# rland93/rrtplanner

Measured on AMD Instinct MI355X. Metric: RRT* nodes-expanded/s on 1024x1024 Perlin grid; achieved HBM GB/s, higher is better.
Workload: dtype int16x2 coordinates / u32 squared distances / f64 costs; 1 GPU; BASELINE.json configs[1]: RRT* 1024x1024 n=50000 r_rewire=64; queries_per_gpu=1, total_queries=1, n=50000, unfinished_queries=0, cus_per_query=129, pipelined=True, team_fallbacks=0, collective_library=librccl.so.1

## Files before the change

### rrtplanner_amd/csrc/kernels_tu.hip

```cpp
#include <hip/hip_runtime.h>

#ifndef RRT_TU
#error "kernels_tu.hip is compiled once per unit: pass -DRRT_TU=k (the Makefile's TUS)"
#endif

#if RRT_TU == 1
#include "rrt_pipe.h"

#elif RRT_TU == 4
#define RRT_PIPE_LARGE_TU
#include "rrt_pipe.h"

#elif RRT_TU == 2
#include "rrt_dubins_block.h"
#include "rrt_serial.h"
namespace rrtdev {
template __global__ void rrt_expand_kernel<false, true>(BatchView);
}

#elif RRT_TU == 3
#include "rrt_serial.h"
namespace rrtdev {
template __global__ void rrt_expand_kernel<false, false>(BatchView);
template __global__ void rrt_expand_kernel<true, false>(BatchView);
// ... 7 lines not shown
#include "rrt_routes.h"

#elif RRT_TU == 7
#include "rrt_keep.h"

#elif RRT_TU == 8
#include "rrt_seed.h"
#include "rrt_pose_seed.h"

#elif RRT_TU == 9
#include "rrt_pose_goals.h"
#include "rrt_pose_keep.h"
#include "rrt_pose_routes.h"

#elif RRT_TU == 0
#include "rrt_reroot.h"
#include "rrt_relax.h"
#include "rrt_pose_relax.h"
#include "rrt_pose_reroot.h"

#elif RRT_TU == -1
#include "rrt_pose_field.h"

#else
#include "rrt_block.h"
namespace rrtdev {
#define K(G, BSM, PIPE, INF) template __global__ void rrt_expand_block_kernel<G, BSM, PIPE, INF>(BatchView);
#define S(G, BSM, INF)                                                        \
    template __global__ void rrt_block_commit_kernel<G, BSM, INF>(BatchView); \
    template __global__ void rrt_block_work_kernel<G, BSM, INF>(BatchView);
#define RRT_PASTE_(a, b) a##b
#define RRT_PASTE(a, b) RRT_PASTE_(a, b)
RRT_PASTE(RRT_UNIT_, RRT_TU)(K, S)
#undef K
#undef S
}
#endif
```

### rrtplanner_amd/csrc/rrt_block.h

```cpp
#pragma once

#include "rrt_go2goal.h"
#include "rrt_cell_stream.h"

namespace rrtdev {

constexpr int BS = 16;

#ifndef RRT_PIPE_LAG
#define RRT_PIPE_LAG 2
#endif
#ifndef RRT_PIPE_LAG_SMALL
#define RRT_PIPE_LAG_SMALL 1
#endif
#ifndef RRT_PIPE_LAG_INF
#define RRT_PIPE_LAG_INF 2
#endif
constexpr unsigned long long TEAM_TIMEOUT_TICKS = 50000000ull;

typedef unsigned long long u64;
typedef __attribute__((address_space(1))) uint32_t gu32;
typedef __attribute__((address_space(1))) u64 gu64;
#define RRT_RLX_AGENT __ATOMIC_RELAXED, __HIP_MEMORY_SCOPE_AGENT

// ... 103 lines not shown
    int32_t i, j, nsoln, vbest_soln, pad0, pad1;
    double cmin_soln, c_ell;
};

template <int BSM>
__device__ __forceinline__ void block_scan_step(u32x4 quad, const uint32_t (&xs16)[BSM], uint32_t (&best)[BSM], uint32_t tag0) {
    const uint32_t n0 = quad.x << 4, n1 = quad.y << 4, n2 = quad.z << 4, n3 = quad.w << 4;
#pragma unroll
    for (int k = 0; k < BSM; ++k) {
        const uint32_t k0 = key16(n0, xs16[k], tag0), k1 = key16(n1, xs16[k], tag0 + 1), k2 = key16(n2, xs16[k], tag0 + 2),
                       k3 = key16(n3, xs16[k], tag0 + 3);
        best[k] = min(min(best[k], k0), min(min(k1, k2), k3));
    }
}

struct GSlot {
    double c1, c2;
    uint32_t i1, i2;
    uint32_t hits, nlist;
    uint32_t nn_d2, nn_idx;
    uint32_t pad[2];
    uint32_t x1, x2;
    uint32_t nn_xy, nn_vlo, nn_vhi;
};
struct GCtl {
    double lbc;
    uint32_t lbi, consume;
    double bound;
};

union BlkWords {
    BlkState b;
    u64 w[5];
};

struct ParRound {
    u64 acc_opt, aprev[NPMAX];
    uint32_t list[NWAVE];
    uint32_t accs[64];
    uint32_t count;
    int32_t jp0[NPMAX];
};

template <bool PIPE, bool INF, int BSM>
struct PipeShape {
    static constexpr int LAG = PIPE ? (INF ? RRT_PIPE_LAG_INF : (BSM >= 16 ? RRT_PIPE_LAG_SMALL : RRT_PIPE_LAG)) : 0;
    static_assert(LAG <= NPMAX, "a record carries masks for NPMAX blocks in flight");
    static constexpr int NP = LAG > 0 ? LAG : 1;
    static constexpr int NSLOT = PIPE ? LAG + 1 : 1;
};

template <int G, int BSM, bool PIPE, bool INF>
struct BlockLds {
    static constexpr int SB = BSM * G, NP = PipeShape<PIPE, INF, BSM>::NP;
    alignas(16) u32x2 nnx[(BSM <= BS ? BSM : 1) * NWAVE];
    alignas(16) BRec brec[PIPE ? 2 : 1][SB];
    uint32_t xq_next[PIPE ? 2 : 1][PIPE ? 64 : 1];
    uint32_t pre_state[2];
    alignas(16) BSlot bslots[2 * NWAVE];
    alignas(16) BlkState blk;
    alignas(16) unsigned long long statred[SB * 5];
    uint32_t xq_lds[SB];
    double newcost[SB];
    alignas(16) ParRound par;
    uint32_t xqp_lds[PIPE ? NP : 1][PIPE ? 64 : 1];
    double prevcost[PIPE ? NP : 1][PIPE ? 64 : 1];
    uint32_t help_n[NWAVE], help_x[NWAVE];
    uint32_t help_any;
    uint32_t tick;
    uint32_t slots[BSM >= 16 ? NWAVE : 1][64];
    alignas(16) GSlot gslot[NWAVE];
    alignas(16) GCtl gctl[BSM];
    alignas(8) uint16_t plist[(PIPE && BSM < 16) ? BSM : 1][PL_MAX];
    uint32_t oq_cnt[(PIPE && BSM < 16) ? BSM : 1], oq_ovf;
    uint32_t qhist[16], qstage2;
#ifdef RRT_STAMPS
    unsigned long long dbg[16];
#endif
};

constexpr int ROLE_ALL = 0, ROLE_COMMIT = 1, ROLE_WORK = 2;


template <int G, int BSM, bool PIPE, bool INF, int ROLE, int CW = NWAVE>
__device__ __forceinline__ void rrt_block_body(BatchView bv, BlockLds<G, BSM, PIPE, INF> &L) {
    static_assert(CW == NWAVE || ROLE == ROLE_COMMIT, "only a committer runs with fewer waves");
    constexpr int NTG = CW * 64;
    static_assert(G >= 1 && G <= TEAM_MAX && BSM >= 1 && BSM * G <= 64, "team size");
    constexpr bool WIDE = BSM > BS;
    static_assert(!PIPE || G > 1, "a pipeline needs a team");
    static_assert(PIPE == (ROLE != ROLE_ALL), "roles are the halves of a pipelined team");
    constexpr int LAG = PipeShape<PIPE, INF, BSM>::LAG, NP = PipeShape<PIPE, INF, BSM>::NP, NSLOT = PipeShape<PIPE, INF, BSM>::NSLOT;
    constexpr int SB = BSM * G;
#ifndef RRT_CG16
#define RRT_CG16 2
#endif
    constexpr int CG = (BSM >= 16) ? (ROLE == ROLE_COMMIT ? 2 : RRT_CG16) : 1;
#ifndef RRT_BLOCK_SCATTER
#define RRT_BLOCK_SCATTER 1
#endif
    constexpr bool SCATTER = RRT_BLOCK_SCATTER && BSM >= 16;
    extern __shared__ __attribute__((aligned(16))) unsigned char smem[];
    auto &nnx = L.nnx;
    auto &brec = L.brec;
    auto &xq_next = L.xq_next;
    auto &pre_state = L.pre_state;
    auto &bslots = L.bslots;
    auto &blk = L.blk;
    auto &statred = L.statred;
    auto &xq_lds = L.xq_lds;
    auto &newcost = L.newcost;
    auto &par = L.par;
    auto &xqp_lds = L.xqp_lds;
    auto &prevcost = L.prevcost;
    auto &gslot = L.gslot;
    auto &gctl = L.gctl;
    constexpr int WPS = BSM >= 16 ? 1 : NWAVE / BSM;
    constexpr bool FASTL = PIPE && WPS > 1;
    const int t = (int)threadIdx.x, lane = t & 63, wave = t >> 6;
    int q = (int)blockIdx.x, g_ = 0;
    if (G > 1) {
        q = (int)blockIdx.x % bv.team_qpad;
        g_ = (int)blockIdx.x / bv.team_qpad + bv.member0;
        if (q >= bv.Q) return;
// ... 44 lines not shown
    const int lds_chunks = bv.lds_chunks;
    const int lds_nodes = lds_chunks * CHUNK;
    const uint32_t r2 = D->r2_rewire, goal_d2 = D->goal_d2;
    const uint32_t xs = pack_xy(D->xs[0], D->xs[1]), xg = pack_xy(D->xg[0], D->xg[1]);
    const int ub_offset = D->ub_offset, ub_count = D->ub_count;
    const int cshift = D->cell_shift, ncy = D->ncy, ccap = D->cell_cap, ncells = D->ncx * D->ncy;
    u32x4 *cellrec = reinterpret_cast<u32x4 *>(bv.cellrec) + (size_t)q * (size_t)bv.rec_stride;
    uint32_t *cellcnt_g = bv.cellcnt + (size_t)q * (size_t)MAX_CELLS;
    const bool cells_on = star || BSM >= 16;
    const uint32_t r2h = star ? r2 : (cells_on ? (uint32_t)((2 << cshift) * (2 << cshift)) : 0u);
    int rad = 0;
    if (r2h > 0) {
        rad = (r2h >= (1u << 23)) ? 4096 : (int)sqrtf((float)(r2h - 1));
        while (rad > 0 && (uint32_t)(rad * rad) > r2h - 1) --rad;
        while ((uint32_t)((rad + 1) * (rad + 1)) <= r2h - 1) ++rad;
    }

    RRT_LDS uint32_t *nodes_lds = (RRT_LDS uint32_t *)smem;
    const RRT_LDS u32x4 *nodes_lds4 = (const RRT_LDS u32x4 *)smem;
    RRT_LDS uint32_t *cellcnt = (RRT_LDS uint32_t *)(smem + (size_t)lds_chunks * CHUNK * sizeof(uint32_t));

    int i = D->i, j = D->j;
    int nsoln = D->nsoln, vbest_soln = D->vbest_soln;
    double cmin_soln = D->cmin_soln;
    int i_switch = D->i_switch;
    int status = ST_RUNNING;
#ifdef RRT_STAMPS
    unsigned long long cyc[6] = {D->cyc[0], D->cyc[1], D->cyc[2], D->cyc[3], D->cyc[4], D->cyc[5]};
    unsigned long long tstamp = __builtin_amdgcn_s_memtime();
    unsigned long long wcyc_acc = 0, wcyc_los = 0;
    auto &dbg = L.dbg;
    if (t < 16) dbg[t] = 0;
    unsigned long long dbgt = __builtin_amdgcn_s_memtime();
#ifdef RRT_STAMPS_LIGHT
#define DBGT(k)                                                      \
    do {                                                             \
        if (((RRT_STAMPS_LIGHT) >> (k)) & 1) {                       \
            unsigned long long now_ = __builtin_amdgcn_s_memtime();  \
            if (t == 0) dbg[k] += now_ - dbgt;                       \
            dbgt = now_;                                             \
        }                                                            \
    } while (0)
#else
#define DBGT(k)                                                  \
    do {                                                         \
        unsigned long long now_ = __builtin_amdgcn_s_memtime();  \
        if (t == 0) dbg[k] += now_ - dbgt;                       \
        dbgt = now_;                                             \
    } while (0)
#endif
#else
#define DBGT(k) \
    do {        \
    } while (0)
#endif

#if defined(RRT_STAMPS)
#define TSMARK(ep, ev)                                                                                          \
    do {                                                                                                        \
        if ((int)(ep) >= RRT_TS_BASE && (int)(ep) < RRT_TS_BASE + 32 && lane == 0) D->ts[((int)(ep) - RRT_TS_BASE) * 16 + (ev)] = wall_clock64(); \
    } while (0)
#else
#define TSMARK(ep, ev) \
    do {               \
    } while (0)
#endif
// ... 137 lines not shown
                    if (base + 3 >= jlim) cur.w = node0;
                }
                block_scan_step<BSA>(cur, xs16, best, (uint32_t)c << 2);
                cur = nxt;
            }
        }
    };

    constexpr int32_t ST_FLAG_RESTART = 1, ST_FLAG_STOP = 2;
    const bool pipe_inf = PIPE && informed;
    int nprev = 0;
    int void_turns = 0;
    bool prefetched = false;
    bool prefetched_smp = false;
    int bsel = 0;
    auto publish_state = [&](uint32_t ep, int32_t flags) {
        if (lane == 0) {
            BlkWords u;
            u.b.i = i;
            u.b.j = j;
            u.b.nsoln = nsoln;
            u.b.vbest_soln = vbest_soln;
            u.b.pad0 = 0;
            u.b.pad1 = flags;
            u.b.cmin_soln = cmin_soln;
            u.b.c_ell = c_ell;
#pragma unroll
            for (int w = 0; w < 5; ++w) __hip_atomic_store(t_state + (size_t)(ep % NSLOT) * 8 + w, u.w[w], RRT_RLX_AGENT);
        }
        asm volatile("s_waitcnt vmcnt(0)" ::: "memory");
        if (lane == 0) __hip_atomic_store(t_go, ep, RRT_RLX_AGENT);
        if (!grid_nn) __builtin_amdgcn_fence(__ATOMIC_ACQUIRE, "agent");
    };
    if (PIPE && SH == 2) {
        if (shift1) {
            if (wave == 0) xqp_lds[0][lane] = (i + lane < n) ? at32(samples, (uint32_t)(i + lane)) : 0u;
            i += SB;
            epoch = 1;
            nprev = 1;
        }
        __syncthreads();
    }
    while ((pipe_inf && g > 0) || i < n) {
        const int i0 = i, j0 = j;
        int nb = (n - i0) < SB ? (n - i0) : SB;
        const bool ell = informed && nsoln > 0;
        bool void_blk = false;
        if (nb <= 0) {
            nb = 0;
            void_blk = true;
        }
        if (ell) {
            if (i_switch == n) i_switch = i0;
            const int u0i = i0 - ub_offset;
            if (ub == nullptr || u0i < 0 || u0i + nb > ub_count) {
                if (pipe_inf && g > 0) {
                    nb = 0;
                    void_blk = true;
                } else {
                    status = ST_NEED_UB;
                    if (pipe_inf && wave == 0) publish_state(epoch + 1, ST_FLAG_STOP);
                    break;
                }
            }
        }
        ++epoch;
// ... 220 lines not shown
        for (int k = 0; k < 16; ++k) D->wcyc[16 * g + k] = dbg[k];
#endif
}

template <int G, int BSM, bool PIPE, bool INF>
__global__ __launch_bounds__(TPB) void rrt_expand_block_kernel(BatchView bv) {
    __shared__ BlockLds<G, BSM, PIPE, INF> L;
    if constexpr (PIPE) {
#if defined(RRT_ONLY_ROLE) && RRT_ONLY_ROLE == 1
        rrt_block_body<G, BSM, PIPE, INF, ROLE_COMMIT>(bv, L);
#elif defined(RRT_ONLY_ROLE) && RRT_ONLY_ROLE == 2
        rrt_block_body<G, BSM, PIPE, INF, ROLE_WORK>(bv, L);
#else
        if ((int)blockIdx.x < bv.team_qpad) rrt_block_body<G, BSM, PIPE, INF, ROLE_COMMIT>(bv, L);
        else rrt_block_body<G, BSM, PIPE, INF, ROLE_WORK>(bv, L);
#endif
    } else {
        rrt_block_body<G, BSM, PIPE, INF, ROLE_ALL>(bv, L);
    }
}

template <int G, int BSM, bool INF>
__global__ __launch_bounds__(512) void rrt_block_commit_kernel(BatchView bv) {
    __shared__ BlockLds<G, BSM, true, INF> L;
    rrt_block_body<G, BSM, true, INF, ROLE_COMMIT, 8>(bv, L);
}

template <int G, int BSM, bool INF>
__global__ __launch_bounds__(TPB) void rrt_block_work_kernel(BatchView bv) {
    __shared__ BlockLds<G, BSM, true, INF> L;
    rrt_block_body<G, BSM, true, INF, ROLE_WORK>(bv, L);
}

}

#include "rrt_block_variants.def"
```

### rrtplanner_amd/csrc/rrt_block_handover.inc

```

        if (PIPE && g > 0) {
#ifdef RRT_STAMPS
            if (t == 0 && g <= 64) {
                const unsigned long long dres = __builtin_amdgcn_s_memtime() - wres0;
                if (dres > 26000ull) D->dbg2[192 + g - 1] += 1;
                if (dres > 32000ull) D->dbg2[256 + g - 1] += 1;
                if (dres > 40000ull) D->dbg2[320 + g - 1] += 1;
                if (dres > D->dbg2[384 + g - 1]) D->dbg2[384 + g - 1] = dres;
            }
#endif
            DBGT(0);
            const int i_next = i0 + nb + (SH - 1) * SB;
            const bool more = i_next < n;
            const uint32_t ep_take = epoch + (uint32_t)(SH - 1) - (uint32_t)LAG;
            const bool take = (int)epoch + SH - 1 > LAG && (more || pipe_inf);
            if (wave == 0) {
                if (!void_blk) {
                    const RRT_LDS u64 *src = (const RRT_LDS u64 *)&brec[0][wg * BSM];
                    gu64 *dst = t_rec + (size_t)(epoch % NSLOT) * 64 * BREC_WORDS + (size_t)wg * BSM * BREC_WORDS;
                    for (int w = lane; w < BSM * BREC_WORDS; w += 64) __hip_atomic_store(dst + w, src[w], RRT_RLX_AGENT);
                    asm volatile("s_waitcnt vmcnt(0)" ::: "memory");
                }
                if (lane == 0) __hip_atomic_store(my_arrive(), epoch, RRT_RLX_AGENT);
                if (g == 1) TSMARK(epoch, 5);
                if (g == 8) TSMARK(epoch, 8);
            }
            pre_i = -1;
            if (!informed && more && !grid_nn) {
                pre_i = i_next;
                pre_j = j0;
                const int nbn = (n - pre_i) < SB ? (n - pre_i) : SB;
                pre_xv = lane < nbn ? at32(samples, (uint32_t)(pre_i + lane)) : 0u;
                uint32_t xsn[BSA];
#pragma unroll
                for (int k = 0; k < BSA; ++k) {
                    const int sk = wg * BSM + k;
                    uint32_t X = (uint32_t)__builtin_amdgcn_readlane((int)pre_xv, sk);
                    if (sk >= nbn) X = (uint32_t)__builtin_amdgcn_readlane((int)pre_xv, 0);
                    xsn[k] = X << 4;
                    pre_best[k] = NONE;
                }
                scan_steps(0, pre_j / CHUNK, pre_j, xsn, pre_best);
            }
            if (wave == 0) {
                bool ok = true;
                if (SH == 2) {
                    xqp_lds[NP - 1][lane] = xv;
                    xqp_lds[0][lane] = more ? at32(samples, (uint32_t)(i0 + nb + lane)) : 0u;
                } else {
#pragma unroll
                    for (int p2 = NP - 1; p2 > 0; --p2) xqp_lds[p2][lane] = xqp_lds[p2 - 1][lane];
                    xqp_lds[0][lane] = xv;
                }
                DBGT(1);
                if (take) {
                    ok = team_wait(t_go, ep_take, t_fail);
                    if (g == 1) TSMARK(epoch, 6);
                    if (g == 8) TSMARK(epoch, 9);
// ... 24 lines not shown
                    if (cells_on) __hip_atomic_fetch_add(&cellcnt[cell_of(Xn)], 1u, __ATOMIC_RELAXED, __HIP_MEMORY_SCOPE_WORKGROUP);
                }
                j = jn;
                if (pipe_inf) {
                    nsoln = unis32(u.b.nsoln);
                    vbest_soln = unis32(u.b.vbest_soln);
                    cmin_soln = unif64(u.b.cmin_soln);
                    c_ell = unif64(u.b.c_ell);
                    if ((u.b.pad1 & ST_FLAG_RESTART) != 0) {
                        __syncthreads();
                        if (wave == 0) {
                            const bool ok2 = team_wait(t_go, epoch, t_fail);
                            if (lane == 0) blk.pad0 = ok2 ? 0 : 1;
                        }
                        __syncthreads();
                        if (blk.pad0 != 0) {
                            team_failed = true;
                            break;
                        }
                        BlkWords u2;
#pragma unroll
                        for (int w = 0; w < 5; ++w) u2.w[w] = __hip_atomic_load(t_state + (size_t)(epoch % NSLOT) * 8 + w, RRT_RLX_AGENT);
                        if ((u2.b.pad1 & ST_FLAG_STOP) != 0) break;
                        i = unis32(u.b.i);
                        nprev = 0;
                    }
                }
            }
            __syncthreads();
            if (wave == 0 && g == 1) TSMARK(epoch, 7);
            if (wave == 0 && g == 8) TSMARK(epoch, 10);
            DBGT(3);
            epoch += (uint32_t)(SH - 1);
            continue;
        }

        if (G > 1 && !PIPE && g > 0) {
            if (wave == 0) {
                const RRT_LDS u64 *src = (const RRT_LDS u64 *)&brec[0][g * BSM];
                for (int w = lane; w < BSM * BREC_WORDS; w += 64) __hip_atomic_store(t_rec + (size_t)g * BSM * BREC_WORDS + w, src[w], RRT_RLX_AGENT);
                asm volatile("s_waitcnt vmcnt(0)" ::: "memory");
                if (lane == 0) __hip_atomic_store(t_arrive + 32 * g, epoch, RRT_RLX_AGENT);
            }
            pre_i = -1;
            if (!informed && i0 + nb < n && !grid_nn) {
                pre_i = i0 + nb;
                pre_j = j0;
                const int nbn = (n - pre_i) < SB ? (n - pre_i) : SB;
                pre_xv = lane < nbn ? samples[pre_i + lane] : 0u;
                uint32_t xsn[BSA];
#pragma unroll
                for (int k = 0; k < BSA; ++k) {
                    const int sk = g * BSM + k;
                    uint32_t X = (uint32_t)__builtin_amdgcn_readlane((int)pre_xv, sk);
                    if (sk >= nbn) X = (uint32_t)__builtin_amdgcn_readlane((int)pre_xv, 0);
                    xsn[k] = X << 4;
                    pre_best[k] = NONE;
                }
                scan_steps(0, pre_j / CHUNK, pre_j, xsn, pre_best);
            }
            if (wave == 0) {
                const bool ok = team_wait(t_go, epoch, t_fail);
                if (!grid_nn) {
                    __builtin_amdgcn_fence(__ATOMIC_ACQUIRE, "agent");
                    asm volatile("s_waitcnt vmcnt(0)" ::: "memory");
                }
// ... 26 lines not shown
```

### rrtplanner_amd/csrc/rrt_block_worker.inc

```

        if (worker && !void_blk) {
        uint32_t xs16[BSA];
#pragma unroll
        for (int k = 0; k < BSA; ++k) {
            const int sk = wg * BSM + k;
            uint32_t X = (uint32_t)__builtin_amdgcn_readlane((int)xv, sk);
            if (sk >= nb) X = (uint32_t)__builtin_amdgcn_readlane((int)xv, 0);
            xs16[k] = X << 4;
        }

        const int nsteps = (j0 + CHUNK - 1) / CHUNK;
        if (!grid_nn) {
            uint32_t best[BSA];
            int c_first = 0;
            if (G > 1 && pre_i == i0) {
                c_first = pre_j / CHUNK;
#pragma unroll
                for (int k = 0; k < BSA; ++k) best[k] = pre_best[k];
            } else {
#pragma unroll
                for (int k = 0; k < BSA; ++k) best[k] = NONE;
            }
            scan_steps(c_first, nsteps, j0, xs16, best);
            uint32_t gd = NONE, gi = NONE;
// ... 378 lines not shown
                            pnn[p2] = __ballot(dp < d2s);
                            pr[p2] = __ballot(star && dp < r2);
                            pdup[p2] = __ballot(xop == Xk);
                        }
                    }
                }
#ifdef RRT_STAMPS
                gs2 = __builtin_amdgcn_s_memtime();
#endif
                if (star) {
                    if (overflow) {
                        nnear = 0;
                        amin = 0.0f;
                        snapshot_parent(Xk, j0, false, cnear_s, pc, pi, nnear, ntests, tcells);
                    } else if (tt.i1 != NONE) {
                        if (!tested3) los_wave2(og, H, tx1, tt.i2 != NONE ? tx2 : Xk, tt.i2 != NONE, Xk, lane, ok1, cc1, ok2, cc2);
                        ntests += 1;
                        tcells += (uint32_t)cc1;
                        if (ok1) {
                            pc = tt.c1;
                            pi = tt.i1;
                        } else if (tt.i2 != NONE) {
                            ntests += 1;
                            tcells += (uint32_t)cc2;
                            if (ok2) {
                                pc = tt.c2;
                                pi = tt.i2;
                            } else {
                                consume = true;
                                lbc = tt.c2;
                                lbi = tt.i2 + 1;
                            }
                        }
                    }
                }
            }
#ifdef RRT_STAMPS
            if (lead) gs3 = __builtin_amdgcn_s_memtime();
#endif
            if (star) {
                if (lead && lane == 0) {
                    GCtl c;
                    c.lbc = lbc;
                    c.lbi = lbi;
                    c.consume = (act && consume) ? 1u : 0u;
                    c.bound = cnear_s;
                    gctl[sl] = c;
                }
                __syncthreads();
                const GCtl c = gctl[sl];
                auto qbin = [](double cn, double lo, double hi) -> int {
                    const double w = hi - lo;
                    if (!(w > 0.0)) return 0;
                    const int b = (int)((cn - lo) * (16.0 / w));
                    return b < 0 ? 0 : (b > 15 ? 15 : b);
                };
                bool by_queue = false;
                if constexpr (GQ) {
                    if (rad < 64) {
                        RRT_LDS u32x4 *const oq = (RRT_LDS u32x4 *)&brec[1][0] + (size_t)sl * OQCAP;
#ifdef RRT_STAMPS
                        unsigned long long qt0 = __builtin_amdgcn_s_memtime(), qt1 = qt0, qt2 = qt0, qt3 = qt0, qt4 = qt0;
#endif
                        if (c.consume != 0u) {
                            const float boundf = screen_of(c.bound);
                            float am = FINF;
// ... 383 lines not shown
```

### rrtplanner_amd/csrc/rrt_engine.hip

```cpp
#include "rrt_engine.h"
#include "rrt_prims.h"

static thread_local std::string g_last_error;

constexpr int RRT_GRID_FAST = 2048;
constexpr int RRT_GRID_LARGE = 4096;
constexpr int RRT_GRID_MAX = 32767;

struct BlockVariant {
    int G, BSM;
    bool pipe, inf;
    block_kernel_fn one, commit, work;
};
static const BlockVariant g_block_variants[] = {
#define K(G, BSM, PIPE, INF) {G, BSM, PIPE, INF, rrt_expand_block_kernel<G, BSM, PIPE, INF>, nullptr, nullptr},
#define S(G, BSM, INF) {G, BSM, true, INF, nullptr, rrt_block_commit_kernel<G, BSM, INF>, rrt_block_work_kernel<G, BSM, INF>},
#define U(k) RRT_UNIT_##k(K, S)
    RRT_BLOCK_UNITS(U)
#undef U
#undef S
#undef K
};

static const BlockVariant *find_variant(int team, bool pipe, bool inf, bool wide, bool split) {
    for (const BlockVariant &r : g_block_variants)
        if (r.G == team && r.pipe == pipe && r.inf == inf && (r.BSM > 16) == wide && (r.commit != nullptr) == split) return &r;
    return nullptr;
}

static size_t block_kernel_static_lds(int team) {
    hipFuncAttributes a{};
    size_t worst = 0;
    for (const BlockVariant &r : g_block_variants)
        for (block_kernel_fn k : {r.one, r.commit, r.work}) {
            if (!k || r.G > team) continue;
            if (hipFuncGetAttributes(&a, reinterpret_cast<const void *>(k)) != hipSuccess) return 16384;
            worst = a.sharedSizeBytes > worst ? a.sharedSizeBytes : worst;
        }
    return (worst + 255) & ~(size_t)255;
}

void drop_keep_views(rrt_batch *b, int32_t q) {
    for (size_t k = 0; k < b->keep_alive.size(); ++k)
        if ((q < 0 || (size_t)q == k) && b->keep_alive[k] >= 0) {
            b->keep_alive[k] = -1;
            b->ran_gen[k] = 0;
            b->ran_og[k] = nullptr;
        }
}

static hipError_t raise_dynamic_lds(int device, const void *kern, int bytes) {
    static std::mutex mu;
    static std::vector<std::tuple<int, const void *, int>> have;
    std::lock_guard<std::mutex> lock(mu);
    for (auto &t : have)
        if (std::get<0>(t) == device && std::get<1>(t) == kern) {
            if (std::get<2>(t) >= bytes) return hipSuccess;
            const hipError_t e = hipFuncSetAttribute(kern, hipFuncAttributeMaxDynamicSharedMemorySize, bytes);
            if (e == hipSuccess) std::get<2>(t) = bytes;
            return e;
        }
    const hipError_t e = hipFuncSetAttribute(kern, hipFuncAttributeMaxDynamicSharedMemorySize, bytes);
    if (e == hipSuccess) have.emplace_back(device, kern, bytes);
    return e;
}

int fail(rrt_ctx *ctx, int code, const char *fmt, ...) {
// ... 771 lines not shown

extern "C" int rrt_batch_launch(rrt_batch *b) {
    if (!b) return fail(nullptr, RRT_E_ARG, "rrt_batch_launch: NULL");
    rrt_ctx *ctx = b->ctx;
    for (int q = 0; q < b->Q; ++q)
        if (b->grow_n[(size_t)q] >= 0 && b->h_desc[(size_t)q].status == ST_RUNNING &&
            (b->grow_gen[(size_t)q] != ctx->grid_gen || b->grow_og[(size_t)q] != ctx->og))
            return fail(ctx, RRT_E_ARG, "rrt_batch_launch: the context's grid was replaced since query %d was seeded by rrt_batch_grow (grid generation %llu then, "
                        "%llu now): its seed belongs to the other grid (rrt_batch_rearm drops the grow)", q, (unsigned long long)b->grow_gen[(size_t)q],
                        (unsigned long long)ctx->grid_gen);
    b->drop_routes();
    drop_keep_views(b);
    if (!ctx->og) return fail(ctx, RRT_E_NOGRID, "rrt_batch_launch: no grid");
    if (b->gridW != ctx->W || b->gridH != ctx->H) return fail(ctx, RRT_E_ARG, "rrt_batch_launch: grid changed shape");
    HIPCHK(ctx, hipSetDevice(ctx->device));
    if (!b->one_cu_once) b->ms_before = 0.f;
    LaunchPlan &p = b->last;
    if (const int rc = plan_launch(b, p); rc != RRT_OK) return rc;
    for (int q = 0; q < b->Q; ++q)
        if (b->h_desc[(size_t)q].status == ST_RUNNING) {
            b->ran_gen[(size_t)q] = ctx->grid_gen;
            b->ran_og[(size_t)q] = ctx->og;
        }
    BatchView v = make_view(b);
    v.team_qpad = p.qpad;
    v.shifts = p.shifts;
    if (p.shifts == 2) v.spill_stride = b->spill_stride2;
    v.lds_chunks = p.lds_chunks;
    if (p.split) {
        if (!ctx->stream2) HIPCHK(ctx, hipStreamCreateWithFlags(&ctx->stream2, hipStreamNonBlocking));
        if (!b->ev_fork) HIPCHK(ctx, hipEventCreateWithFlags(&b->ev_fork, hipEventDisableTiming));
        if (!b->ev_join) HIPCHK(ctx, hipEventCreateWithFlags(&b->ev_join, hipEventDisableTiming));
    }
    for (block_kernel_fn k : {p.kern, p.split ? p.row->commit : nullptr, p.split ? p.row->work : nullptr})
        if (k && p.lds_bytes) HIPCHK(ctx, raise_dynamic_lds(ctx->device, reinterpret_cast<const void *>(k), (int)p.lds_bytes));
    const dim3 ig((unsigned)((b->bitmap_words + 255) / 256 > 64 ? 64 : (b->bitmap_words + 255) / 256), (unsigned)b->Q);
    hipLaunchKernelGGL(rrt_init_kernel<0>, ig, dim3(256), 0, ctx->stream, v);
    if (p.team > 1) HIPCHK(ctx, hipMemsetAsync(b->d_team, 0, (size_t)b->Q * TEAM_BYTES, ctx->stream));
    HIPCHK(ctx, hipEventRecord(b->ev0, ctx->stream));
    if (p.split) {
        HIPCHK(ctx, hipEventRecord(b->ev_fork, ctx->stream));
        HIPCHK(ctx, hipStreamWaitEvent(ctx->stream2, b->ev_fork, 0));
        hipLaunchKernelGGL(p.row->commit, dim3((unsigned)p.qpad), dim3(512), p.lds_bytes, ctx->stream2, v);
        BatchView vw = v;
        vw.member0 = 1;
        hipLaunchKernelGGL(p.row->work, dim3((unsigned)(p.qpad * p.team * p.shifts)), dim3(TPB), p.lds_bytes, ctx->stream, vw);
        HIPCHK(ctx, hipEventRecord(b->ev_join, ctx->stream2));
        HIPCHK(ctx, hipStreamWaitEvent(ctx->stream, b->ev_join, 0));
    } else {
        hipLaunchKernelGGL(p.kern, dim3(p.grid), dim3(TPB), p.lds_bytes, ctx->stream, v);
    }
    HIPCHK(ctx, hipEventRecord(b->ev1, ctx->stream));
    HIPCHK(ctx, hipGetLastError());
    b->timed = true;
    return RRT_OK;
}

extern "C" int rrt_batch_sync(rrt_batch *b) {
    if (!b) return fail(nullptr, RRT_E_ARG, "rrt_batch_sync: NULL");
    rrt_ctx *ctx = b->ctx;
    HIPCHK(ctx, hipSetDevice(ctx->device));
    HIPCHK(ctx, hipMemcpyAsync(b->h_desc.data(), b->d_desc, (size_t)b->Q * sizeof(QDesc), hipMemcpyDeviceToHost, ctx->stream));
    HIPCHK(ctx, wait_stream_spin(ctx->stream));
    cu_release(ctx->device, b->claimed_cus);
    b->claimed_cus = 0;
#ifdef RRT_STAMPS
    if (getenv("RRT_STAMPS_DUMP")) {
        const QDesc &d0 = b->h_desc[0];
        fprintf(stderr, "dbg2 groups of slow blocks (> 32 k) [count, own stream, first barrier, nearest + LoS, top-2 LoS, tail, consume, empty ball]:");
        for (int m = 0; m < 8; ++m) fprintf(stderr, " %llu", d0.dbg2[m]);
        fprintf(stderr, "\ndbg2 groups of the other blocks:");
        for (int m = 8; m < 16; ++m) fprintf(stderr, " %llu", d0.dbg2[m]);
        fprintf(stderr, "\ndbg2 groups queue, fast [count, gctl barrier, pricing, barrier, tests, barrier, queue entries, time before]:");
        for (int m = 16; m < 24; ++m) fprintf(stderr, " %llu", d0.dbg2[m]);
        fprintf(stderr, "\ndbg2 groups queue, slow (> 30 k at the last barrier):");
        for (int m = 24; m < 32; ++m) fprintf(stderr, " %llu", d0.dbg2[m]);
        fprintf(stderr, "\ndbg2 missing-polls:");
        for (int m = 0; m < 64; ++m) fprintf(stderr, " %llu", d0.dbg2[m]);
        fprintf(stderr, "\ndbg2 last-to-arrive:");
// ... 713 lines not shown
```

### rrtplanner_amd/csrc/rrt_kernel_abi.h

```cpp
#pragma once

#include <hip/hip_runtime.h>
#include <stddef.h>
#include <stdint.h>

namespace rrtdev {

constexpr int TPB = 1024;
constexpr int NWAVE = TPB / 64;
constexpr int CHUNK = TPB * 4;
constexpr int MAX_LDS_CHUNKS = 8;
constexpr int WSLOTS = 3;
constexpr int WCAP = 64 * WSLOTS;
constexpr uint32_t NONE = 0xffffffffu;

typedef uint32_t u32x4 __attribute__((ext_vector_type(4)));

#ifndef RRT_TS_BASE
#define RRT_TS_BASE 300
#endif

enum : int32_t { ST_DONE = 0, ST_NEED_UB = 1, ST_UNREACHABLE = -2, ST_TEAM_FAIL = -3, ST_RUNNING = 100, ST_IDLE = 101 };

struct QDesc {
// ... 376 lines not shown
    uint8_t *item_h;
    int32_t x0, y0, w, h;
    int32_t heading_lo, heading_hi;
    int32_t run;
    int32_t *vertex;
    double *cost;
    int32_t *heading_out;
};
enum : int { POSE_FIELD_CELLS = 0, POSE_FIELD_BUCKETS_SEEN = 1, POSE_FIELD_WORDS = 2, POSE_FIELD_SWEEPS = 3, POSE_FIELD_STATS = 4 };

struct PoseRerootView {
    const uint32_t *nodes;
    const int32_t *parent;
    const uint8_t *heading;
    const int32_t *id;
    int32_t j, root;
    uint32_t *f_nodes;
    int32_t *f_parent;
    uint8_t *f_heading;
    int32_t *f_id;
};

template <bool RW, bool DUB = false>
__global__ __launch_bounds__(TPB) void rrt_expand_kernel(BatchView bv);
__global__ __launch_bounds__(TPB) void rrt_pipe_kernel(BatchView bv);
__global__ __launch_bounds__(TPB) void rrt_pipe_large_kernel(BatchView bv);
__global__ __launch_bounds__(TPB) void rrt_dubins_block_kernel(BatchView bv);
template <int G, int BSM, bool PIPE, bool INF>
__global__ __launch_bounds__(TPB) void rrt_expand_block_kernel(BatchView bv);
template <int G, int BSM, bool INF>
__global__ __launch_bounds__(512) void rrt_block_commit_kernel(BatchView bv);
template <int G, int BSM, bool INF>
__global__ __launch_bounds__(TPB) void rrt_block_work_kernel(BatchView bv);
__global__ __launch_bounds__(TPB) void rrt_goals_kernel(GoalsView gv);
__global__ __launch_bounds__(TPB) void rrt_goals_large_kernel(GoalsView gv);
__global__ __launch_bounds__(TPB) void rrt_pose_goals_kernel(PoseGoalsView pv);
__global__ __launch_bounds__(FIELD_TPB) void rrt_field_kernel(FieldView fv);
__global__ __launch_bounds__(FIELD_TPB) void rrt_field_large_kernel(FieldView fv);
__global__ __launch_bounds__(ROUTE_TPB) void rrt_route_depth_kernel(RoutesView rv);
__global__ __launch_bounds__(TPB) void rrt_route_scan_kernel(const int32_t *in, int64_t *out, int32_t m);
__global__ __launch_bounds__(ROUTE_TPB) void rrt_route_fill_kernel(RoutesView rv, int32_t with_len);
__global__ __launch_bounds__(TPB) void rrt_route_cut_kernel(RoutesView rv);
__global__ __launch_bounds__(TPB) void rrt_route_cut_large_kernel(RoutesView rv);
__global__ __launch_bounds__(ROUTE_TPB) void rrt_route_pack_kernel(RoutesView rv);
__global__ __launch_bounds__(KEEP_TPB) void rrt_keep_edge_kernel(KeepView kv);
__global__ __launch_bounds__(KEEP_TPB) void rrt_keep_edge_large_kernel(KeepView kv);
__global__ __launch_bounds__(KEEP_TPB) void rrt_keep_jump_kernel(const uint8_t *ok, const int32_t *anc, uint8_t *ok2, int32_t *anc2, int32_t j);
__global__ __launch_bounds__(TPB) void rrt_keep_compact_kernel(KeepCompact kc);
__global__ __launch_bounds__(KEEP_TPB) void rrt_keep_remap_kernel(int32_t *vertex, const int32_t *live_id, int32_t m, int32_t count);
__global__ __launch_bounds__(POSE_KEEP_TPB) void rrt_pose_keep_edge_kernel(PoseKeepView kv);
__global__ __launch_bounds__(POSE_KEEP_TPB) void rrt_pose_keep_gather_kernel(const uint8_t *heading, const int32_t *live_id, const int32_t *count,
                                                                            uint8_t *live_heading, int32_t j);
__global__ __launch_bounds__(POSE_ROUTE_TPB) void rrt_pose_route_fill_kernel(PoseRoutesView pr);
__global__ __launch_bounds__(POSE_ROUTE_TPB) void rrt_pose_route_leg_kernel(PoseRoutesView pr);
__global__ __launch_bounds__(POSE_ROUTE_TPB) void rrt_pose_route_length_kernel(PoseRoutesView pr);
__global__ __launch_bounds__(POSE_ROUTE_TPB) void rrt_pose_route_points_kernel(PoseRoutesView pr);
__global__ __launch_bounds__(POSE_CUT_TPB) void rrt_pose_route_cut_kernel(PoseCutView pc);
__global__ __launch_bounds__(POSE_CUT_TPB) void rrt_pose_route_pack_kernel(PoseCutView pc);
__global__ __launch_bounds__(SEED_TPB) void rrt_seed_rank_kernel(SeedView sv);
__global__ __launch_bounds__(SEED_TPB) void rrt_seed_parent_kernel(SeedView sv);
__global__ __launch_bounds__(SEED_TPB) void rrt_seed_install_kernel(SeedView sv);
__global__ __launch_bounds__(SEED_TPB) void rrt_seed_bitmap_kernel(SeedView sv);
__global__ __launch_bounds__(SEED_TPB) void rrt_seed_records_kernel(SeedRecords sr);
__global__ __launch_bounds__(SEED_TPB) void rrt_pose_seed_heading_kernel(uint8_t *heading, const uint8_t *live_heading, int32_t j0, int32_t node_stride);

__global__ __launch_bounds__(REROOT_TPB) void rrt_reroot_path_kernel(RerootView rv);
// ... 34 lines not shown
```

Baseline: 6.664 million nodes/s.

## Let split-team workers resolve ahead and patch results after the committer catches up

Adds a work-ahead variant of the pipelined worker kernel for the 64-member, BSM=1, non-informed split team. Workers take the next sample without waiting for the committer's state. When the committed state arrives, they patch their nearest/parent/rewire record using the newly inserted nodes, with a small LOS batch. If the patch cannot be done cheaply (too many new nodes, hard constraint, or overflow), they redo the block. The host picks this kernel when the rewire radius is between 16 and 64. The aim is to hide committer latency, at the cost of extra catch-up work and possible redo rounds.

```diff
diff --git a/rrtplanner_amd/csrc/kernels_tu.hip b/rrtplanner_amd/csrc/kernels_tu.hip
--- a/rrtplanner_amd/csrc/kernels_tu.hip
+++ b/rrtplanner_amd/csrc/kernels_tu.hip
@@ -63,6 +63,9 @@
 #define RRT_PASTE_(a, b) a##b
 #define RRT_PASTE(a, b) RRT_PASTE_(a, b)
 RRT_PASTE(RRT_UNIT_, RRT_TU)(K, S)
+#if RRT_TU == 22
+template __global__ void rrt_block_work_ahead_kernel<TEAM_MAX, 1, false>(BatchView);
+#endif
 #undef K
 #undef S
 }
diff --git a/rrtplanner_amd/csrc/rrt_block.h b/rrtplanner_amd/csrc/rrt_block.h
--- a/rrtplanner_amd/csrc/rrt_block.h
+++ b/rrtplanner_amd/csrc/rrt_block.h
@@ -159,6 +159,17 @@
 union BlkWords {
     BlkState b;
     u64 w[5];
+};
+
+constexpr uint32_t AH_T1 = 1u, AH_T2 = 2u;
+constexpr uint32_t AH_HARD = 4u;
+constexpr uint32_t AH_OVERFLOW = 8u;
+struct AheadSlot {
+    double c1, c2;
+    uint32_t i1, i2;
+    uint32_t cc1, cc2;
+    uint32_t st;
+    uint32_t redo;
 };
 
 struct ParRound {
@@ -209,7 +220,7 @@
 constexpr int ROLE_ALL = 0, ROLE_COMMIT = 1, ROLE_WORK = 2;
 
 
-template <int G, int BSM, bool PIPE, bool INF, int ROLE, int CW = NWAVE>
+template <int G, int BSM, bool PIPE, bool INF, int ROLE, int CW = NWAVE, bool AHEAD = false>
 __device__ __forceinline__ void rrt_block_body(BatchView bv, BlockLds<G, BSM, PIPE, INF> &L) {
     static_assert(CW == NWAVE || ROLE == ROLE_COMMIT, "only a committer runs with fewer waves");
     constexpr int NTG = CW * 64;
@@ -217,6 +228,7 @@
     constexpr bool WIDE = BSM > BS;
     static_assert(!PIPE || G > 1, "a pipeline needs a team");
     static_assert(PIPE == (ROLE != ROLE_ALL), "roles are the halves of a pipelined team");
+    static_assert(!AHEAD || (ROLE == ROLE_WORK && !INF && BSM == 1 && G == TEAM_MAX), "only the workers of the split team of 64 resolve ahead");
     constexpr int LAG = PipeShape<PIPE, INF, BSM>::LAG, NP = PipeShape<PIPE, INF, BSM>::NP, NSLOT = PipeShape<PIPE, INF, BSM>::NSLOT;
     constexpr int SB = BSM * G;
 #ifndef RRT_CG16
@@ -327,6 +339,7 @@
     auto &dbg = L.dbg;
     if (t < 16) dbg[t] = 0;
     unsigned long long dbgt = __builtin_amdgcn_s_memtime();
+    [[maybe_unused]] unsigned long long ah_go = 0;
 #ifdef RRT_STAMPS_LIGHT
 #define DBGT(k)                                                      \
     do {                                                             \
@@ -530,6 +543,10 @@
         if (lane == 0) __hip_atomic_store(t_go, ep, RRT_RLX_AGENT);
         if (!grid_nn) __builtin_amdgcn_fence(__ATOMIC_ACQUIRE, "agent");
     };
+    const bool ahead = AHEAD && SH == 2 && grid_nn && rad < 64;
+    bool early = false;
+    static_assert(!AHEAD || sizeof(AheadSlot) <= sizeof(L.newcost), "the catch-up's notes fit the committer's cost array");
+    [[maybe_unused]] RRT_LDS AheadSlot *const ah = AHEAD ? (RRT_LDS AheadSlot *)&newcost[0] : nullptr;
     if (PIPE && SH == 2) {
         if (shift1) {
             if (wave == 0) xqp_lds[0][lane] = (i + lane < n) ? at32(samples, (uint32_t)(i + lane)) : 0u;
@@ -816,6 +833,12 @@
     rrt_block_body<G, BSM, true, INF, ROLE_WORK>(bv, L);
 }
 
+template <int G, int BSM, bool INF>
+__global__ __launch_bounds__(TPB) void rrt_block_work_ahead_kernel(BatchView bv) {
+    __shared__ BlockLds<G, BSM, true, INF> L;
+    rrt_block_body<G, BSM, true, INF, ROLE_WORK, NWAVE, true>(bv, L);
+}
+
 }
 
 #include "rrt_block_variants.def"
diff --git a/rrtplanner_amd/csrc/rrt_block_handover.inc b/rrtplanner_amd/csrc/rrt_block_handover.inc
--- a/rrtplanner_amd/csrc/rrt_block_handover.inc
+++ b/rrtplanner_amd/csrc/rrt_block_handover.inc
@@ -10,10 +10,224 @@
             }
 #endif
             DBGT(0);
+            if constexpr (AHEAD) {
+                if (early) {
+                    early = false;
+                    if ((int)epoch - 1 > LAG) {
+                        const uint32_t ep_due = epoch - 1u - (uint32_t)LAG;
+                        DBGT(1);
+                        if (wave == 0) {
+                            const bool ok = team_wait(t_go, ep_due, t_fail);
+                            if (lane == 0) blk.pad0 = ok ? 0 : 1;
+                        }
+                        __syncthreads();
+                        DBGT(2);
+#ifdef RRT_STAMPS
+                        ah_go = __builtin_amdgcn_s_memtime();
+#endif
+                        if (blk.pad0 != 0) {
+                            team_failed = true;
+                            break;
+                        }
+                        BlkWords u;
+#pragma unroll
+                        for (int w = 0; w < 5; ++w) u.w[w] = __hip_atomic_load(t_state + (size_t)(ep_due % NSLOT) * 8 + w, RRT_RLX_AGENT);
+                        const int jn = unis32(u.b.j);
+                        if (t < jn - j0) {
+                            const uint32_t Xn = ld_u32<COH>(&at32(nodes_g, (uint32_t)(j0 + t)));
+                            if (j0 + t < lds_nodes) nodes_lds[j0 + t] = Xn;
+                            if (cells_on) __hip_atomic_fetch_add(&cellcnt[cell_of(Xn)], 1u, __ATOMIC_RELAXED, __HIP_MEMORY_SCOPE_WORKGROUP);
+                        }
+                        j = jn;
+                        if (wave == 0) {
+                            const int sidx = wg * BSM;
+                            const uint32_t Xk = (uint32_t)__builtin_amdgcn_readlane((int)xv, sidx);
+                            BRec &r = brec[0][sidx];
+                            const uint32_t st = uni32(ah->st);
+                            const int m = sidx < nb ? jn - j0 : 0;
+                            uint32_t redo = (m > 128 || (m > 0 && (st & AH_OVERFLOW) != 0u)) ? 1u : 0u;
+#ifdef RRT_STAMPS
+                            uint32_t lost = 0;
+#endif
+                            if (m > 0 && redo == 0u) {
+                                const uint32_t id0 = (uint32_t)(j0 + lane), id1 = id0 + 64u;
+                                const bool v0 = (int)id0 < jn, v1 = (int)id1 < jn;
+                                const uint32_t X0 = ld_u32<COH>(&at32(nodes_g, v0 ? id0 : 0u)), X1 = ld_u32<COH>(&at32(nodes_g, v1 ? id1 : 0u));
+                                const double V0 = ld_f64<COH>(&at32(vcost, v0 ? id0 : 0u)), V1 = ld_f64<COH>(&at32(vcost, v1 ? id1 : 0u));
+                                const uint32_t e0 = dist2(X0, Xk), e1 = dist2(X1, Xk);
+                                const bool dupn = __ballot((v0 && X0 == Xk) || (v1 && X1 == Xk)) != 0;
+                                uint32_t kd = v0 ? e0 : NONE, ki = v0 ? id0 : NONE;
+                                if (v1 && e1 < kd) {
+                                    kd = e1;
+                                    ki = id1;
+                                }
+                                wave_min_key_idx(kd, ki);
+                                uint32_t d2s = uni32(r.d2s), vs = uni32(r.vs), los_s = uni32(r.los_s), nnear = uni32(r.nnear);
+                                double Vs = unif64(r.Vs), pc = unif64(r.pc);
+                                uint32_t pi = pc < f64_inf() ? uni32(r.vbest) : NONE;
+                                float amin = __uint_as_float(uni32(__float_as_uint(r.amin)));
+                                const uint32_t ps0 = uni32(r.pstat);
+                                const double B0 = Vs + sqrt_u24(d2s);
+                                const bool changed = kd < d2s;
+                                uint32_t vsxy = Xk;
+                                if (changed) {
+                                    if (kd >= r2h || (st & AH_HARD) != 0u) {
+                                        redo = 1u;
+                                    } else {
+                                        const bool p1 = ki - (uint32_t)j0 >= 64u;
+                                        const int ln_ = (int)((ki - (uint32_t)j0) & 63u);
+                                        const u64 vb = (u64)__double_as_longlong(p1 ? V1 : V0);
+                                        vsxy = (uint32_t)__builtin_amdgcn_readlane((int)(p1 ? X1 : X0), ln_);
+                                        Vs = __longlong_as_double((long long)(((u64)(uint32_t)__builtin_amdgcn_readlane((int)(uint32_t)(vb >> 32), ln_) << 32) |
+                                                                              (uint32_t)__builtin_amdgcn_readlane((int)(uint32_t)vb, ln_)));
+                                        d2s = kd;
+                                        vs = ki;
+                                    }
+                                }
+                                const double B = Vs + sqrt_u24(d2s);
+                                const bool h0 = v0 && e0 < r2h, h1 = v1 && e1 < r2h;
+                                const double c0 = V0 + sqrt_u24(e0), c1 = V1 + sqrt_u24(e1);
+                                uint32_t ntests = ps0 >> 20, tcells = ps0 & 0xfffffu;
+                                if (star && redo == 0u) {
+                                    nnear += (uint32_t)__builtin_popcountll(__ballot(h0)) + (uint32_t)__builtin_popcountll(__ballot(h1));
+                                    if (B > B0 && pi == NONE && !((double)amin >= B)) redo = 1u;
+                                    if (pi != NONE && !(pc < B)) {
+                                        pi = NONE;
+                                        pc = f64_inf();
+                                    }
+                                }
+                                if (star && redo == 0u) {
+                                    const bool q0 = h0 && c0 < B && key_lt(c0, id0, pc, pi), q1 = h1 && c1 < B && key_lt(c1, id1, pc, pi);
+                                    u64 s0 = __ballot(q0), s1 = __ballot(q1);
+                                    const int nq = __builtin_popcountll(s0) + __builtin_popcountll(s1);
+                                    if (nq > LOSB - 1) {
+                                        redo = 1u;
+                                    } else {
+                                        uint32_t res0 = 0x80000000u, res1 = 0x80000000u;
+                                        if (changed || nq != 0) {
+                                            uint32_t a8[LOSB];
+                                            int l8[LOSB];
+                                            a8[0] = vsxy;
+                                            l8[0] = -1;
+#pragma unroll
+                                            for (int q8 = 1; q8 < LOSB; ++q8) {
+                                                a8[q8] = Xk;
+                                                l8[q8] = -1;
+                                                if (s0) {
+                                                    l8[q8] = (int)__builtin_ctzll(s0);
+                                                    s0 &= s0 - 1;
+                                                    a8[q8] = (uint32_t)__builtin_amdgcn_readlane((int)X0, l8[q8]);
+                                                } else if (s1) {
+                                                    const int l_ = (int)__builtin_ctzll(s1);
+                                                    s1 &= s1 - 1;
+                                                    a8[q8] = (uint32_t)__builtin_amdgcn_readlane((int)X1, l_);
+                                                    l8[q8] = 64 + l_;
+                                                }
+                                            }
+                                            bool ok8[LOSB];
+                                            int cells8[LOSB];
+                                            los_batch(og, H, a8, 1 + nq, Xk, lane, ok8, cells8);
+                                            if (changed) los_s = (ok8[0] ? 0x80000000u : 0u) | (uint32_t)cells8[0];
+#pragma unroll
+                                            for (int q8 = 1; q8 < LOSB; ++q8) {
+                                                const uint32_t rs = (uint32_t)cells8[q8] | (ok8[q8] ? 0u : 0x80000000u);
+                                                if (l8[q8] == lane) res0 = rs;
+                                                if (l8[q8] == 64 + lane) res1 = rs;
+                                            }
+#ifdef RRT_STAMPS
+                                            lost = 1;
+#endif
+                                        }
+                                        double wc = f64_inf();
+                                        uint32_t wi = NONE;
+                                        if (q0 && (res0 >> 31) == 0u) {
+                                            wc = c0;
+                                            wi = id0;
+                                        }
+                                        if (q1 && (res1 >> 31) == 0u && key_lt(c1, id1, wc, wi)) {
+                                            wc = c1;
+                                            wi = id1;
+                                        }
+                                        wave_min_f64_idx(wc, wi);
+                                        if (wi != NONE) {
+                                            pc = wc;
+                                            pi = wi;
+                                        }
+                                        if ((st & AH_HARD) != 0u) {
+                                            if (wi != NONE) redo = 1u;
+                                        } else {
+                                            const double a1 = unif64(ah->c1), a2 = unif64(ah->c2);
+                                            const uint32_t b1 = uni32(ah->i1), b2 = uni32(ah->i2);
+                                            const bool t1 = (st & AH_T1) != 0u && a1 < B && (pi == NONE || !key_lt(pc, pi, a1, b1));
+                                            const bool t2 = (st & AH_T2) != 0u && a2 < B && (pi == NONE || !key_lt(pc, pi, a2, b2));
+                                            ntests = (t1 ? 1u : 0u) + (t2 ? 1u : 0u);
+                                            tcells = (t1 ? uni32(ah->cc1) : 0u) + (t2 ? uni32(ah->cc2) : 0u);
+                                        }
+                                        const bool n0 = q0 && (wi == NONE || !key_lt(wc, wi, c0, id0)), n1 = q1 && (wi == NONE || !key_lt(wc, wi, c1, id1));
+                                        ntests += wave_sum_u32((n0 ? 1u : 0u) + (n1 ? 1u : 0u));
+                                        tcells += wave_sum_u32((n0 ? res0 & 0x7fffffffu : 0u) + (n1 ? res1 & 0x7fffffffu : 0u));
+                                        if (B < B0) {
+                                            amin = lower_f32(B);
+                                        } else {
+                                            float an = FINF;
+                                            if (h0 && !(c0 < B)) an = lower_f32(c0);
+                                            if (h1 && !(c1 < B)) an = __builtin_fminf(an, lower_f32(c1));
+                                            an = wave_min_f32_nonneg(an);
+                                            amin = amin == 0.0f ? 0.0f : __builtin_fminf(amin, an);
+                                        }
+                                    }
+                                }
+                                if (redo == 0u) {
+                                    u64 nnm = 0, pnn_[NP] = {};
+                                    if (changed) {
+                                        const uint32_t xo = (lane < sidx) ? xq_lds[lane] : Xk;
+                                        nnm = __ballot(lane < sidx && dist2(xo, Xk) < d2s);
+#pragma unroll
+                                        for (int p2 = 0; p2 < NP; ++p2)
+                                            if (p2 < nprev) pnn_[p2] = __ballot(dist2(xqp_lds[p2][lane], Xk) < d2s);
+                                    }
+                                    if (lane == 0) {
+                                        r.d2s = d2s;
+                                        r.vs = vs;
+                                        r.los_s = los_s;
+                                        if (dupn) r.flags |= 1u;
+                                        r.Vs = Vs;
+                                        r.cbest = (pi != NONE) ? pc : B;
+                                        r.vbest = (pi != NONE) ? pi : vs;
+                                        r.pstat = (ntests << 20) | (tcells & 0xfffffu);
+                                        r.nnear = nnear;
+                                        r.amin = amin;
+                                        r.pc = pc;
+                                        if (changed) {
+                                            r.nnmask = nnm;
+#pragma unroll
+                                            for (int p2 = 0; p2 < NP; ++p2) r.pnn[p2] = pnn_[p2];
+                                        }
+                                    }
+                                }
+                            }
+                            if (lane == 0) ah->redo = redo;
+#ifdef RRT_STAMPS
+                            if (lane == 0) {
+                                dbg[12] += 1;
+                                dbg[13] += lost;
+                                dbg[14] += redo;
+                            }
+#endif
+                        }
+                        __syncthreads();
+                        if (uni32(ah->redo) != 0u) {
+                            --epoch;
+                            continue;
+                        }
+                    }
+                }
+            }
             const int i_next = i0 + nb + (SH - 1) * SB;
             const bool more = i_next < n;
+            const bool go_ahead = AHEAD && ahead && more;
             const uint32_t ep_take = epoch + (uint32_t)(SH - 1) - (uint32_t)LAG;
-            const bool take = (int)epoch + SH - 1 > LAG && (more || pipe_inf);
+            const bool take = !go_ahead && (int)epoch + SH - 1 > LAG && (more || pipe_inf);
             if (wave == 0) {
                 if (!void_blk) {
                     const RRT_LDS u64 *src = (const RRT_LDS u64 *)&brec[0][wg * BSM];
@@ -24,6 +238,10 @@
                 if (lane == 0) __hip_atomic_store(my_arrive(), epoch, RRT_RLX_AGENT);
                 if (g == 1) TSMARK(epoch, 5);
                 if (g == 8) TSMARK(epoch, 8);
+#ifdef RRT_STAMPS
+                if (lane == 0 && ah_go != 0ull) dbg[15] += __builtin_amdgcn_s_memtime() - ah_go;
+                ah_go = 0ull;
+#endif
             }
             pre_i = -1;
             if (!informed && more && !grid_nn) {
@@ -114,6 +332,7 @@
             if (wave == 0 && g == 8) TSMARK(epoch, 10);
             DBGT(3);
             epoch += (uint32_t)(SH - 1);
+            if (AHEAD && go_ahead) early = true;
             continue;
         }
 
diff --git a/rrtplanner_amd/csrc/rrt_block_worker.inc b/rrtplanner_amd/csrc/rrt_block_worker.inc
--- a/rrtplanner_amd/csrc/rrt_block_worker.inc
+++ b/rrtplanner_amd/csrc/rrt_block_worker.inc
@@ -434,6 +434,18 @@
                                 lbi = tt.i2 + 1;
                             }
                         }
+                    }
+                }
+                if constexpr (AHEAD) {
+                    if (lane == 0) {
+                        const bool t1 = star && !overflow && tt.i1 != NONE, t2 = t1 && !ok1 && tt.i2 != NONE;
+                        ah->c1 = tt.c1;
+                        ah->c2 = tt.c2;
+                        ah->i1 = tt.i1;
+                        ah->i2 = tt.i2;
+                        ah->cc1 = (uint32_t)cc1;
+                        ah->cc2 = (uint32_t)cc2;
+                        ah->st = (t1 ? AH_T1 : 0u) | (t2 ? AH_T2 : 0u) | (consume ? AH_HARD : 0u) | (overflow ? AH_OVERFLOW : 0u);
                     }
                 }
             }
diff --git a/rrtplanner_amd/csrc/rrt_engine.hip b/rrtplanner_amd/csrc/rrt_engine.hip
--- a/rrtplanner_amd/csrc/rrt_engine.hip
+++ b/rrtplanner_amd/csrc/rrt_engine.hip
@@ -11,10 +11,16 @@
     int G, BSM;
     bool pipe, inf;
     block_kernel_fn one, commit, work;
+    block_kernel_fn ahead;
 };
+template <int G, int BSM, bool INF>
+static constexpr block_kernel_fn work_ahead_of() {
+    if constexpr (G == TEAM_MAX && BSM == 1 && !INF) return rrt_block_work_ahead_kernel<G, BSM, INF>;
+    else return nullptr;
+}
 static const BlockVariant g_block_variants[] = {
-#define K(G, BSM, PIPE, INF) {G, BSM, PIPE, INF, rrt_expand_block_kernel<G, BSM, PIPE, INF>, nullptr, nullptr},
-#define S(G, BSM, INF) {G, BSM, true, INF, nullptr, rrt_block_commit_kernel<G, BSM, INF>, rrt_block_work_kernel<G, BSM, INF>},
+#define K(G, BSM, PIPE, INF) {G, BSM, PIPE, INF, rrt_expand_block_kernel<G, BSM, PIPE, INF>, nullptr, nullptr, nullptr},
+#define S(G, BSM, INF) {G, BSM, true, INF, nullptr, rrt_block_commit_kernel<G, BSM, INF>, rrt_block_work_kernel<G, BSM, INF>, work_ahead_of<G, BSM, INF>()},
 #define U(k) RRT_UNIT_##k(K, S)
     RRT_BLOCK_UNITS(U)
 #undef U
@@ -32,7 +38,7 @@
     hipFuncAttributes a{};
     size_t worst = 0;
     for (const BlockVariant &r : g_block_variants)
-        for (block_kernel_fn k : {r.one, r.commit, r.work}) {
+        for (block_kernel_fn k : {r.one, r.commit, r.work, r.ahead}) {
             if (!k || r.G > team) continue;
             if (hipFuncGetAttributes(&a, reinterpret_cast<const void *>(k)) != hipSuccess) return 16384;
             worst = a.sharedSizeBytes > worst ? a.sharedSizeBytes : worst;
@@ -870,7 +876,17 @@
         if (!b->ev_fork) HIPCHK(ctx, hipEventCreateWithFlags(&b->ev_fork, hipEventDisableTiming));
         if (!b->ev_join) HIPCHK(ctx, hipEventCreateWithFlags(&b->ev_join, hipEventDisableTiming));
     }
-    for (block_kernel_fn k : {p.kern, p.split ? p.row->commit : nullptr, p.split ? p.row->work : nullptr})
+    block_kernel_fn work = p.split ? p.row->work : nullptr;
+    if (p.split && p.shifts == 2 && p.row->ahead) {
+        bool fits = true;
+        for (int q = 0; q < b->Q; ++q) {
+            const QDesc &d = b->h_desc[(size_t)q];
+            if (d.status != ST_RUNNING) continue;
+            fits = fits && d.alg >= 1 && (int64_t)d.r2_rewire > 16 * 16 && (int64_t)d.r2_rewire <= 64 * 64;
+        }
+        if (fits) work = p.row->ahead;
+    }
+    for (block_kernel_fn k : {p.kern, p.split ? p.row->commit : nullptr, work})
         if (k && p.lds_bytes) HIPCHK(ctx, raise_dynamic_lds(ctx->device, reinterpret_cast<const void *>(k), (int)p.lds_bytes));
     const dim3 ig((unsigned)((b->bitmap_words + 255) / 256 > 64 ? 64 : (b->bitmap_words + 255) / 256), (unsigned)b->Q);
     hipLaunchKernelGGL(rrt_init_kernel<0>, ig, dim3(256), 0, ctx->stream, v);
@@ -882,7 +898,7 @@
         hipLaunchKernelGGL(p.row->commit, dim3((unsigned)p.qpad), dim3(512), p.lds_bytes, ctx->stream2, v);
         BatchView vw = v;
         vw.member0 = 1;
-        hipLaunchKernelGGL(p.row->work, dim3((unsigned)(p.qpad * p.team * p.shifts)), dim3(TPB), p.lds_bytes, ctx->stream, vw);
+        hipLaunchKernelGGL(work, dim3((unsigned)(p.qpad * p.team * p.shifts)), dim3(TPB), p.lds_bytes, ctx->stream, vw);
         HIPCHK(ctx, hipEventRecord(b->ev_join, ctx->stream2));
         HIPCHK(ctx, hipStreamWaitEvent(ctx->stream, b->ev_join, 0));
     } else {
diff --git a/rrtplanner_amd/csrc/rrt_kernel_abi.h b/rrtplanner_amd/csrc/rrt_kernel_abi.h
--- a/rrtplanner_amd/csrc/rrt_kernel_abi.h
+++ b/rrtplanner_amd/csrc/rrt_kernel_abi.h
@@ -432,6 +432,8 @@
 __global__ __launch_bounds__(512) void rrt_block_commit_kernel(BatchView bv);
 template <int G, int BSM, bool INF>
 __global__ __launch_bounds__(TPB) void rrt_block_work_kernel(BatchView bv);
+template <int G, int BSM, bool INF>
+__global__ __launch_bounds__(TPB) void rrt_block_work_ahead_kernel(BatchView bv);
 __global__ __launch_bounds__(TPB) void rrt_goals_kernel(GoalsView gv);
 __global__ __launch_bounds__(TPB) void rrt_goals_large_kernel(GoalsView gv);
 __global__ __launch_bounds__(TPB) void rrt_pose_goals_kernel(PoseGoalsView pv);
```

Result: faster. 7.047 million nodes/s (median of 6 runs) (+5.7%).
